# Ryan-Faulkner/Simultaneous-Diffusion-for-Pointclouds

Measured on AMD Instinct MI355X. Metric: Langevin denoising steps/sec on 64×1024 range images, 1/2/4/8 MI355X, higher is better.
Workload: dtype fp32x3; 1 GPU; Line.yml simultaneous sampling step (score-net fwd + Langevin update + consistency merge), 64x1024x2 range images; views_per_gpu=4, megabatch_views=4, mode=viewsplit, conv_arithmetic=fp32x3, parallelism=views1

## Files before the change

### simultaneous-diffusion-for-pointclouds_amd/csrc/conv_kernel.h

```cpp
#pragma once
#include <type_traits>

#include "common.h"

namespace sdp {

#ifndef SDP_KO
#define SDP_KO 0
#endif

#ifndef SDP_DMA_AUX
#define SDP_DMA_AUX 0
#endif
#ifndef SDP_STORE_AUX
#define SDP_STORE_AUX 0
#endif
#ifndef SDP_STORE_AUX16
#define SDP_STORE_AUX16 SDP_STORE_AUX
#endif

#ifndef SDP_S2_RING
#define SDP_S2_RING 4
#endif

#ifdef SDP_TIMING
#define SDP_T(i) do { if (tid == 0) tclk[i] = __builtin_amdgcn_s_memtime(); } while (0)
#else
#define SDP_T(i) do { } while (0)
#endif

constexpr int PSTRIDE = 144;

template <int WM, int TC, int KS, int NW = 4, int NJ = 4, bool IO16 = false>
struct ConvTile {
  static constexpr int NTH = 64 * NW;
  static constexpr int WN = NW / WM;
  static constexpr int RW = 128 / TC;
  static constexpr int TR = WM * RW;
  static constexpr int NTILE = WN * 16 * NJ;
  static constexpr int WPC = 4 * (NJ == 2 ? 2 : 1) / NW;
  static constexpr int HALO = KS == 3 ? 1 : 0;
  static constexpr int PC = TC + 2 * HALO;
  static constexpr int PR = TR + 2 * HALO;
  static constexpr int NPIX = PR * PC;
  static constexpr int UPP = IO16 ? 4 : 8;
  static constexpr int NU = (NPIX * UPP + NTH - 1) / NTH;
  static constexpr int PATCH_BYTES = NU * (NTH / UPP) * PSTRIDE;
  static constexpr int RAW_BYTES = NU * NTH * 16;
  static constexpr int PIPE_BYTES = 2 * PATCH_BYTES + RAW_BYTES;
  static constexpr int EPI_BYTES = WM * 64 * (NTILE + 8) * 4;
  static constexpr int LDS_BYTES = PIPE_BYTES > EPI_BYTES ? PIPE_BYTES : EPI_BYTES;
  static_assert(LDS_BYTES * WPC <= 160 * 1024, "LDS budget (WPC workgroups per CU)");
};

SDP_DEV float4 ld4(const float* p) { return *reinterpret_cast<const float4*>(p); }

template <int NU, int NT, int NSTG_ = 5>
struct XformPlan {
  static constexpr int tap_of(int k) { return k * NT / NU; }
  static constexpr int first(int tap) {
    int k = 0;
    while (k < NU && tap_of(k) < tap) ++k;
    return k;
  }
  static constexpr int count(int tap) {
    int n = 0;
    for (int k = 0; k < NU; ++k) n += tap_of(k) == tap ? 1 : 0;
    return n;
  }
  static constexpr int max_count() {
    int m = 0;
    for (int t = 0; t < NT; ++t) m = count(t) > m ? count(t) : m;
    return m;
  }
  static constexpr int NSTG = NSTG_;
  static constexpr int stage_blk(int q, int Q, int NBLK) { return 2 + q * (NBLK - 2) / (Q > 0 ? Q : 1); }
};

constexpr int s2_pos(int phase, int t) {
  const int rho = phase >> 1, gamma = phase & 1;
  return ((rho ? 0 : 1) + (t >> 1)) * 3 + (gamma ? 0 : 1) + (t & 1);
}

template <int MODE, int WM, int TC, int KS, bool POOL, bool ZP, bool PELU, int SH = 32, int NW = 4, bool TRN = false,
          int NJ = 4, bool IO16 = false, bool S2 = false>
__global__ __launch_bounds__(64 * NW, NJ == 2 ? 2 : 1) void conv_mfma_kernel(ConvArgs a) {
#if defined(__HIP_DEVICE_COMPILE__)
  static_assert(!IO16 || MODE == MODE_BF16, "the bf16 tape runs in bf16 mode");
  constexpr int ES = IO16 ? 2 : 4;
  constexpr int CPU = IO16 ? 8 : 4;
  constexpr int USH = IO16 ? 2 : 3;
  constexpr int PPU = CPU / 2;
  constexpr bool COPY = IO16 && !PELU;
  static_assert((SH == 32) == (MODE == MODE_F32), "bf16 modes: 16x16 shape; exact fp32: 32x32");
  static_assert(NW == 4 || (SH == 16 && !POOL), "2-wave workgroups: the 16x16 non-pooled forward only");
  static_assert(NJ == 4 || (SH == 16 && !POOL && KS == 3 && WM == 1), "32-Cout waves: the 16x16 3x3 tiles only");
  static_assert(!S2 || (NJ == 2 && NW == 4 && TC == 16 && ZP && !TRN && !IO16), "4x4 stride-2: zero-padded 32-Cout-wave tiles");
  using T = ConvTile<WM, TC, KS, NW, NJ, IO16>;
  constexpr int NTH = T::NTH;
  constexpr int NT = S2 ? 4 : KS * KS;
  constexpr bool TRANS = TRN && SH == 16 && !POOL;
  constexpr int NU = T::NU;
  constexpr int XT = NT >= 4 ? 4 : NT;
  __shared__ __attribute__((aligned(16))) char lds[T::LDS_BYTES];
  char* const raw = lds + 2 * T::PATCH_BYTES;

  const int tid = threadIdx.x, lane = tid & 63, wave = tid >> 6;
#ifdef SDP_TIMING
  unsigned long long tclk[8] = {0, 0, 0, 0, 0, 0, 0, 0};
  unsigned long long tbar = 0;
  const unsigned long long rt0 = __builtin_amdgcn_s_memrealtime();
#endif
  SDP_T(0);
  const int wm = WM == 1 ? 0 : (wave & 1), wn = WM == 1 ? wave : (wave >> 1);
  const int d = S2 ? 2 : a.dil, Hs = a.H / d, Ws = a.W / d;
  const int tiles_c = Ws / TC, tiles_rc = (Hs / T::TR) * tiles_c;
  const int nwg = gridDim.x;
  int t = (nwg & 7) ? (int)blockIdx.x : ((int)blockIdx.x & 7) * (nwg >> 3) + ((int)blockIdx.x >> 3);
  const int cblk = a.cpair ? (t & 1) : (int)blockIdx.y;
  if (a.cpair) t >>= 1;
  const int b = t / a.tiles_per_img;
  const int tile = t - b * a.tiles_per_img;
  t = tile;
  const int ph = t / tiles_rc;
  t -= ph * tiles_rc;
  const int ph_r = ph / d, ph_c = ph - (ph / d) * d;
  int trow, tcol;
  if (a.strip_w) {
    const int R = Hs / T::TR, sw = a.strip_w;
    const int strip = t / (R * sw), w_ = t - strip * (R * sw);
    trow = w_ / sw;
    tcol = strip * sw + (w_ - trow * sw);
  } else {
    trow = t / tiles_c;
    tcol = t % tiles_c;
  }
  const int sr0 = trow * T::TR, sc0 = tcol * TC;
  const int n0 = cblk * T::NTILE;
  const int wrow0 = wm * T::RW;

  const int Cin = a.Cin, Cout = a.Cout;
  const int nck = Cin / 32;
  const int nchunks = S2 ? 4 * nck : nck;
  const int NB = Cout / 32;
  const int f0 = n0 / 16 + wn * NJ;
  const int nbg0 = f0 / 2;

  f32x16 acc[4][2];
  f32x4 acc4[8][NJ];
  if constexpr (SH == 32) {
    static_for<0, 4>([&](auto i) {
      static_for<0, 2>([&](auto j) {
#pragma unroll
        for (int r = 0; r < 16; ++r) acc[i][j][r] = 0.f;
      });
    });
  } else {
    static_for<0, 8>([&](auto i) {
      static_for<0, NJ>([&](auto j) {
#pragma unroll
        for (int r = 0; r < 4; ++r) acc4[i][j][r] = 0.f;
      });
    });
  }

  const bool c16 = SH == 16 && a.wf16 != nullptr;
  const __amdgpu_buffer_rsrc_t wrs =
      __builtin_amdgcn_make_buffer_rsrc((void*)(c16 ? a.wf16 : a.wf), 0, 0x7fffffff, 0x00020000);
  const int wv0 = ((nbg0 + 0) * 64 + lane) * 64, wv1 = ((nbg0 + 1) * 64 + lane) * 64;
  typedef __attribute__((ext_vector_type(4))) unsigned u32x4;
  constexpr int NBUF = S2 ? SDP_S2_RING : (NT % 3 == 0) ? 3 : 2;
  uint4 bq[NBUF][NJ / 2][4];
  int wq16[NJ];
  const int wlo16 = __builtin_amdgcn_readfirstlane(c16 ? 1024 : 16);
  {
    const int g = lane >> 4, h = g & 1, sg = g >> 1;
    static_for<0, NJ>([&](auto njc) {
      constexpr int nj = decltype(njc)::value;
      const int L = 16 * (nj & 1) + (lane & 15) + 32 * h;
      wq16[nj] = c16 ? ((f0 + nj) * 128 + lane) * 16 : ((nbg0 + (nj >> 1)) * 64 + L) * 64 + sg * 32;
    });
  }
  auto load_b = [&](auto buf, int chunk, int tap) __attribute__((always_inline)) {
    constexpr int J = decltype(buf)::value;
    if constexpr (SDP_KO & 4) return;
    const int so = __builtin_amdgcn_readfirstlane(((chunk * NT + tap) * NB) * 4096);
    if constexpr (SH == 32) {
      static_for<0, 4>([&](auto q) {
        const u32x4 v0 = __builtin_amdgcn_raw_buffer_load_b128(wrs, wv0 + q * 16, so, 0);
        const u32x4 v1 = __builtin_amdgcn_raw_buffer_load_b128(wrs, wv1 + q * 16, so, 0);
        bq[J][0][q] = make_uint4(v0.x, v0.y, v0.z, v0.w);
        bq[J][1][q] = make_uint4(v1.x, v1.y, v1.z, v1.w);
      });
    } else {
      static_for<0, NJ>([&](auto njc) {
        constexpr int nj = decltype(njc)::value;
        const u32x4 vh = __builtin_amdgcn_raw_buffer_load_b128(wrs, wq16[nj], so, 0);
        bq[J][nj >> 1][2 * (nj & 1)] = make_uint4(vh.x, vh.y, vh.z, vh.w);
        if constexpr (MODE != MODE_BF16) {
          const u32x4 vl = __builtin_amdgcn_raw_buffer_load_b128(wrs, wq16[nj] + wlo16, so, 0);
          bq[J][nj >> 1][2 * (nj & 1) + 1] = make_uint4(vl.x, vl.y, vl.z, vl.w);
        }
      });
    }
  };

  const char* inb = reinterpret_cast<const char*>(a.in) + (size_t)b * a.H * a.W * Cin * ES;
  const float* ssb = a.pro_ss + (size_t)b * a.ss_bstride;
  auto chunk_cc = [&](int c) __attribute__((always_inline)) {
    if constexpr (S2) return (c >= 2 * nck ? c - 2 * nck : c) >> 1;
    else return c;
  };
  auto chunk_soff = [&](int c) __attribute__((always_inline)) {
    if constexpr (S2) {
      c = min(c, nchunks - 1);
      const int rho = c >= 2 * nck ? 1 : 0, r = c - rho * 2 * nck;
      return ((rho * a.W + (r & 1)) * Cin + (r >> 1) * 32) * ES;
    } else {
      return c * 32 * ES;
    }
  };
  const int my_cv = tid & (T::UPP - 1);
  float4 ssv[2][PPU];
  auto load_ss = [&](auto buf, int chunk) __attribute__((always_inline)) {
    constexpr int SB = decltype(buf)::value;
    static_for<0, PPU>([&](auto kc) { ssv[SB][kc] = ld4(ssb + (chunk * 32 + my_cv * CPU) * 2 + 4 * decltype(kc)::value); });
  };

  const __amdgpu_buffer_rsrc_t irs =
      __builtin_amdgcn_make_buffer_rsrc((void*)inb, 0, a.H * a.W * Cin * ES, 0x00020000);
  int uoff[NU];
  unsigned uvalid = 0;
  static_for<0, NU>([&](auto kc) {
    constexpr int k = decltype(kc)::value;
    int u = tid + k * NTH;
    bool valid = u < T::NPIX * T::UPP;
    u = valid ? u : 0;
    const int pix = u >> USH, cv = u & (T::UPP - 1);
    const int pr = pix / T::PC, pc = pix - pr * T::PC;
    int sr = sr0 - T::HALO + pr, sc = sc0 - T::HALO + pc;
    if (a.circular) {
      sr = sr < 0 ? sr + Hs : (sr >= Hs ? sr - Hs : sr);
      sc = sc < 0 ? sc + Ws : (sc >= Ws ? sc - Ws : sc);
    } else {
      valid = valid && sr >= 0 && sr < Hs && sc >= 0 && sc < Ws;
      sr = min(max(sr, 0), Hs - 1);
      sc = min(max(sc, 0), Ws - 1);
    }
    const int y = sr * d + ph_r, x = sc * d + ph_c;
    uoff[k] = ((y * a.W + x) * Cin + cv * CPU) * ES;
    uvalid |= (valid ? 1u : 0u) << k;
  });
  auto load_unit = [&](auto kc, int chunk) __attribute__((always_inline)) {
    constexpr int k = decltype(kc)::value;
    if constexpr (SDP_KO & 1) return;
    const int base = __builtin_amdgcn_readfirstlane(((tid & ~63) + k * NTH) * 16);
    __builtin_amdgcn_raw_ptr_buffer_load_lds(
        irs, reinterpret_cast<__attribute__((address_space(3))) void*>(reinterpret_cast<uintptr_t>(raw + base)), 16,
        uoff[k], chunk_soff(chunk), 0, SDP_DMA_AUX);
  };
  const i32x4 irs_o = buffer_desc(inb, (uint32_t)(a.H * a.W * Cin * ES));
  auto load_unit_o = [&](auto kc, int chunk) __attribute__((always_inline)) {
    constexpr int k = decltype(kc)::value;
    if constexpr (SDP_KO & 1) return;
    const uint32_t base = (uint32_t)(uintptr_t)(raw + ((tid & ~63) + k * NTH) * 16);
    dma16_lds_opaque(irs_o, base, uoff[k], chunk_soff(chunk));
  };
  auto xform_load = [&](auto kc) __attribute__((always_inline)) {
    constexpr int k = decltype(kc)::value;
    return *reinterpret_cast<const float4*>(raw + (tid + k * NTH) * 16);
  };
  auto xform_store = [&](auto kc, auto pb, float4 v) __attribute__((always_inline)) {
    constexpr int k = decltype(kc)::value;
    constexpr int PB = decltype(pb)::value;
    const int pix = (tid + k * NTH) >> USH;
    if constexpr (COPY) {
      uint4 u = __builtin_bit_cast(uint4, v);
      if constexpr (ZP) {
        if (!((uvalid >> k) & 1u)) u = make_uint4(0u, 0u, 0u, 0u);
      }
      *reinterpret_cast<uint4*>(lds + PB * T::PATCH_BYTES + pix * PSTRIDE + my_cv * 16) = u;
      return;
    }
    if constexpr (IO16) {
      const uint4 u = __builtin_bit_cast(uint4, v);
      const float4 lo = bf4_to_f4(make_uint2(u.x, u.y)), hi = bf4_to_f4(make_uint2(u.z, u.w));
      float x8[8] = {lo.x, lo.y, lo.z, lo.w, hi.x, hi.y, hi.z, hi.w};
#pragma unroll
      for (int e = 0; e < 8; ++e) {
        const float4 sv = ssv[PB][e >> 1];
        x8[e] = fmaf(x8[e], (e & 1) ? sv.z : sv.x, (e & 1) ? sv.w : sv.y);
        if constexpr (PELU) x8[e] = elu_max(x8[e]);
        if constexpr (ZP) {
          if (!((uvalid >> k) & 1u)) x8[e] = 0.f;
        }
      }
      *reinterpret_cast<uint4*>(lds + PB * T::PATCH_BYTES + pix * PSTRIDE + my_cv * 16) =
          make_uint4(pack_bf2(x8[0], x8[1]), pack_bf2(x8[2], x8[3]), pack_bf2(x8[4], x8[5]), pack_bf2(x8[6], x8[7]));
      return;
    }
    const float4 ssv0 = ssv[PB][0], ssv1 = ssv[PB][1];
    v.x = fmaf(v.x, ssv0.x, ssv0.y);
    v.y = fmaf(v.y, ssv0.z, ssv0.w);
    v.z = fmaf(v.z, ssv1.x, ssv1.y);
    v.w = fmaf(v.w, ssv1.z, ssv1.w);
    if constexpr (PELU) {
      v.x = elu_max(v.x); v.y = elu_max(v.y); v.z = elu_max(v.z); v.w = elu_max(v.w);
    }
    if constexpr (ZP) {
      if (!((uvalid >> k) & 1u)) v = make_float4(0.f, 0.f, 0.f, 0.f);
    }
    char* dst = lds + PB * T::PATCH_BYTES + pix * PSTRIDE;
    if constexpr (MODE == MODE_F32) {
      *reinterpret_cast<float4*>(dst + my_cv * 16) = v;
    } else {
      bf16x4 hi;
      hi[0] = (__bf16)v.x; hi[1] = (__bf16)v.y; hi[2] = (__bf16)v.z; hi[3] = (__bf16)v.w;
      *reinterpret_cast<bf16x4*>(dst + my_cv * 8) = hi;
      if constexpr (MODE == MODE_F32X3) {
        bf16x4 lo;
        lo[0] = (__bf16)(v.x - (float)hi[0]);
        lo[1] = (__bf16)(v.y - (float)hi[1]);
        lo[2] = (__bf16)(v.z - (float)hi[2]);
        lo[3] = (__bf16)(v.w - (float)hi[3]);
        *reinterpret_cast<bf16x4*>(dst + 64 + my_cv * 8) = lo;
      }
    }
  };
  auto xform_unit = [&](auto kc, auto pb) __attribute__((always_inline)) { xform_store(kc, pb, xform_load(kc)); };
  auto xform_piece = [&](auto kc, auto hc, auto pb, float4 v4) __attribute__((always_inline)) {
    constexpr int k = decltype(kc)::value, h = decltype(hc)::value, PB = decltype(pb)::value;
    if constexpr (SDP_KO & 2) return;
    const int pix = (tid + k * NTH) >> USH;
    float x0, x1;
    if constexpr (IO16) {
      const uint32_t w = __float_as_uint(h == 0 ? v4.x : h == 1 ? v4.y : h == 2 ? v4.z : v4.w);
      x0 = __uint_as_float(w << 16);
      x1 = __uint_as_float(w & 0xffff0000u);
    } else {
      x0 = h ? v4.z : v4.x;
      x1 = h ? v4.w : v4.y;
    }
    const float4 sv = ssv[PB][h];
    x0 = fmaf(x0, sv.x, sv.y);
    x1 = fmaf(x1, sv.z, sv.w);
    if constexpr (PELU) {
      x0 = elu_max(x0);
      x1 = elu_max(x1);
    }
    if constexpr (ZP) {
      const bool ok = (uvalid >> k) & 1u;
      x0 = ok ? x0 : 0.f;
      x1 = ok ? x1 : 0.f;
    }
    typedef __attribute__((ext_vector_type(2))) __bf16 bf16x2;
    bf16x2 hi;
    hi[0] = (__bf16)x0;
    hi[1] = (__bf16)x1;
    char* dst = lds + PB * T::PATCH_BYTES + pix * PSTRIDE + my_cv * (2 * CPU) + h * 4;
    *reinterpret_cast<bf16x2*>(dst) = hi;
    if constexpr (MODE == MODE_F32X3) {
      bf16x2 lo;
      lo[0] = (__bf16)(x0 - (float)hi[0]);
      lo[1] = (__bf16)(x1 - (float)hi[1]);
      *reinterpret_cast<bf16x2*>(dst + 64) = lo;
    }
  };

  SDP_T(1);
  load_b(std::integral_constant<int, 0>{}, 0, 0);
  static_for<1, NBUF - 1>([&](auto j) { load_b(j, 0, decltype(j)::value); });
  load_ss(std::integral_constant<int, 0>{}, 0);
  static_for<0, NU>([&](auto k) { load_unit(k, 0); });
  static_for<0, NU>([&](auto k) { xform_unit(k, std::integral_constant<int, 0>{}); });
  if (nchunks > 1) {
    load_ss(std::integral_constant<int, 1>{}, chunk_cc(1));
    static_for<0, NU>([&](auto k) { load_unit(k, 1); });
  }
  __syncthreads();
  SDP_T(2);

  const int a_lane_off16 = (lane & 15) * PSTRIDE + (lane >> 4) * 16;
  auto read_a = [&](const char* pat, auto tap_c, auto s_c, bf16x8* hi, bf16x8* lo) __attribute__((always_inline)) {
    constexpr int tap = decltype(tap_c)::value, s = decltype(s_c)::value;
    constexpr int kh = (KS == 3) ? tap / 3 : 0, kw = (KS == 3) ? tap % 3 : 0;
    static_for<0, 4>([&](auto mbc) {
      constexpr int i = decltype(mbc)::value, mb = 4 * s + i;
      constexpr int mr = mb / (TC / 16), mc = (mb % (TC / 16)) * 16;
      const char* src = pat + ((wrow0 + mr + kh) * T::PC + mc + kw) * PSTRIDE + a_lane_off16;
      hi[i] = *reinterpret_cast<const bf16x8*>(src);
      if constexpr (MODE == MODE_F32X3) lo[i] = *reinterpret_cast<const bf16x8*>(src + 64);
    });
  };

  auto do_chunk = [&](auto parity, int chunk) __attribute__((always_inline)) {
    constexpr int P = decltype(parity)::value;
    const char* pat = lds + P * T::PATCH_BYTES;
    bf16x8 pre_hi[4], pre_lo[4];
    if constexpr (MODE != MODE_F32) read_a(pat, std::integral_constant<int, 0>{}, std::integral_constant<int, 0>{},
                                           pre_hi, pre_lo);
    static_for<0, NT>([&](auto tap_c) {
      constexpr int tap = decltype(tap_c)::value;
      constexpr int DIST = NBUF - 1;
      constexpr int CUR = NBUF >= 3 ? tap % NBUF : (tap + P) & 1;
      constexpr int NXT = NBUF >= 3 ? (tap + DIST) % NBUF : (tap + 1 + P) & 1;
      if constexpr (tap + DIST < NT) load_b(std::integral_constant<int, NXT>{}, chunk, tap + DIST);
      else load_b(std::integral_constant<int, NXT>{}, min(chunk + 1, nchunks - 1), tap + DIST - NT);
      __builtin_amdgcn_sched_barrier(0);
      constexpr int NX = (tap < XT) ? (NU - tap + XT - 1) / XT : 0;
      float4 xv[NX > 0 ? NX : 1];
      auto xform_loads = [&]() __attribute__((always_inline)) {
        static_for<0, NX>([&](auto j) { xv[j] = xform_load(std::integral_constant<int, tap + XT * j>{}); });
      };
      auto xform_stores = [&]() __attribute__((always_inline)) {
        static_for<0, NX>([&](auto j) {
          xform_store(std::integral_constant<int, tap + XT * j>{}, std::integral_constant<int, 1 - P>{}, xv[j]);
        });
      };
      auto dmas = [&]() __attribute__((always_inline)) {
        if constexpr (tap == NT - 1) load_ss(std::integral_constant<int, P>{}, min(chunk + 2, nchunks - 1));
        static_for<0, NU>([&](auto kc) {
          constexpr int dt = NT > XT ? XT : 0;
          if constexpr (dt == tap) load_unit(kc, chunk + 2);
        });
      };
      if constexpr (MODE == MODE_F32) {
        xform_loads();
        xform_stores();
        if constexpr (NT == 1) __builtin_amdgcn_sched_barrier(0);
        dmas();
        const int kh = (KS == 3) ? tap / 3 : 0, kw = (KS == 3) ? tap % 3 : 0;
#pragma unroll
        for (int half = 0; half < 2; ++half) {
          float av[4][8];
          static_for<0, 4>([&](auto mbc) {
            constexpr int mb = decltype(mbc)::value;
            constexpr int mr = mb / (TC / 32), mc = (mb % (TC / 32)) * 32;
            const int pix = (wrow0 + mr + kh) * T::PC + mc + (lane & 31) + kw;
            const char* src = pat + pix * PSTRIDE + (lane >> 5) * 64 + half * 32;
            const float4 f0 = *reinterpret_cast<const float4*>(src);
            const float4 f1 = *reinterpret_cast<const float4*>(src + 16);
            av[mb][0] = f0.x; av[mb][1] = f0.y; av[mb][2] = f0.z; av[mb][3] = f0.w;
            av[mb][4] = f1.x; av[mb][5] = f1.y; av[mb][6] = f1.z; av[mb][7] = f1.w;
          });
#pragma unroll
          for (int kk = 0; kk < 8; ++kk) {
            const int k = half * 8 + kk;
            static_for<0, 2>([&](auto nbc) {
              constexpr int nb = decltype(nbc)::value;
              const uint4 bv = bq[CUR][nb][k >> 2];
              const uint32_t bw = (k & 3) == 0 ? bv.x : (k & 3) == 1 ? bv.y : (k & 3) == 2 ? bv.z : bv.w;
              const float bf = __uint_as_float(bw);
              static_for<0, 4>([&](auto mbc) {
                constexpr int mb = decltype(mbc)::value;
                acc[mb][nb] = __builtin_amdgcn_mfma_f32_32x32x2f32(av[mb][kk], bf, acc[mb][nb], 0, 0, 0);
              });
            });
          }
        }
      } else {
        float4 xv[NX > 0 ? NX : 1];
        static_for<0, NX>([&](auto j) { xv[j] = xform_load(std::integral_constant<int, tap + XT * j>{}); });
        bf16x8 c0_hi[4], c0_lo[4], c1_hi[4], c1_lo[4];
        static_for<0, 4>([&](auto mb) {
          c0_hi[mb] = pre_hi[mb];
          if constexpr (MODE == MODE_F32X3) c0_lo[mb] = pre_lo[mb];
        });
        read_a(pat, tap_c, std::integral_constant<int, 1>{}, c1_hi, c1_lo);
        if constexpr (tap + 1 < NT)
          read_a(pat, std::integral_constant<int, tap + 1>{}, std::integral_constant<int, 0>{}, pre_hi, pre_lo);
        if constexpr (NT > 1) dmas();
        constexpr int NBLK = 8 * NJ;
        static_for<0, NBLK>([&](auto blk_c) {
          constexpr int blk = decltype(blk_c)::value;
          {
            constexpr int s = blk / (4 * NJ), nj = (blk / 4) % NJ, i = blk & 3, mb = 4 * s + i;
            const uint4 h4 = bq[CUR][nj >> 1][2 * (nj & 1)], l4 = bq[CUR][nj >> 1][2 * (nj & 1) + 1];
            const bf16x8 bhi = *reinterpret_cast<const bf16x8*>(&h4);
            const bf16x8 blo = *reinterpret_cast<const bf16x8*>(&l4);
            const bf16x8 ahi = s == 0 ? c0_hi[i] : c1_hi[i];
            if constexpr (TRANS) {
              if constexpr (MODE == MODE_F32X3) {
                const bf16x8 alo = s == 0 ? c0_lo[i] : c1_lo[i];
                acc4[mb][nj] = __builtin_amdgcn_mfma_f32_16x16x32_bf16(bhi, alo, acc4[mb][nj], 0, 0, 0);
                acc4[mb][nj] = __builtin_amdgcn_mfma_f32_16x16x32_bf16(blo, ahi, acc4[mb][nj], 0, 0, 0);
              }
              acc4[mb][nj] = __builtin_amdgcn_mfma_f32_16x16x32_bf16(bhi, ahi, acc4[mb][nj], 0, 0, 0);
            } else {
              if constexpr (MODE == MODE_F32X3) {
                const bf16x8 alo = s == 0 ? c0_lo[i] : c1_lo[i];
                acc4[mb][nj] = __builtin_amdgcn_mfma_f32_16x16x32_bf16(alo, bhi, acc4[mb][nj], 0, 0, 0);
                acc4[mb][nj] = __builtin_amdgcn_mfma_f32_16x16x32_bf16(ahi, blo, acc4[mb][nj], 0, 0, 0);
              }
              acc4[mb][nj] = __builtin_amdgcn_mfma_f32_16x16x32_bf16(ahi, bhi, acc4[mb][nj], 0, 0, 0);
            }
          }
          if constexpr (COPY) {
            if constexpr (blk < NX) xform_store(std::integral_constant<int, tap + XT * blk>{}, std::integral_constant<int, 1 - P>{},
                                                xv[blk]);
          } else if constexpr (blk < PPU * NX) {
            xform_piece(std::integral_constant<int, tap + XT * (blk / PPU)>{}, std::integral_constant<int, blk % PPU>{},
                        std::integral_constant<int, 1 - P>{}, xv[blk / PPU]);
          }
          __builtin_amdgcn_sched_barrier(0);
        });
        if constexpr (NT == 1) dmas();
      }
    });
#ifdef SDP_TIMING
    const unsigned long long tb0 = __builtin_amdgcn_s_memtime();
#endif
    __builtin_amdgcn_s_waitcnt(0xc07f);
    if constexpr (!(SDP_KO & 8)) __builtin_amdgcn_s_barrier();
#ifdef SDP_TIMING
    tbar += __builtin_amdgcn_s_memtime() - tb0;
#endif
  };
  using XP = XformPlan<NU, NT, (MODE == MODE_BF16 && !IO16 && !S2) ? 8 : 5>;
  constexpr int NQ = MODE == MODE_F32X3 ? 8 : 4;
  constexpr int NWL = NJ * (MODE == MODE_F32X3 ? 2 : 1);
  constexpr int NBLK = 8 * NJ;
  static_assert(NQ <= NBLK / 2 && 2 * NWL <= NBLK, "the tap's fillers fit its blocks");
  using I0 = std::integral_constant<int, 0>;
  using I1 = std::integral_constant<int, 1>;
  auto read_a1 = [&](const char* pat, auto pos_c, auto s_c, auto i_c, auto lo_c) __attribute__((always_inline)) {
    constexpr int pos = decltype(pos_c)::value, s = decltype(s_c)::value, i = decltype(i_c)::value;
    constexpr int kh = pos / 3, kw = pos % 3, mb = 4 * s + i;
    constexpr int mr = mb / (TC / 16), mc = (mb % (TC / 16)) * 16;
    return *reinterpret_cast<const bf16x8*>(pat + ((wrow0 + mr + kh) * T::PC + mc + kw) * PSTRIDE + a_lane_off16 +
                                            (decltype(lo_c)::value ? 64 : 0));
  };
  auto load_b1 = [&](auto buf, auto q_c, int chunk, int tap) __attribute__((always_inline)) {
    constexpr int J = decltype(buf)::value, q = decltype(q_c)::value;
    constexpr int nj = MODE == MODE_F32X3 ? (q >> 1) : q, part = MODE == MODE_F32X3 ? (q & 1) : 0;
    if constexpr (SDP_KO & 4) return;
    const int so = __builtin_amdgcn_readfirstlane(((chunk * NT + tap) * NB) * 4096 + (part ? wlo16 : 0));
    const u32x4 v = __builtin_amdgcn_raw_buffer_load_b128(wrs, wq16[nj], so, 0);
    bq[J][nj >> 1][2 * (nj & 1) + part] = make_uint4(v.x, v.y, v.z, v.w);
  };
  auto do_chunk9 = [&](auto parity, auto phase_c, int chunk) __attribute__((always_inline)) {
    constexpr int P = decltype(parity)::value, PHS = decltype(phase_c)::value;
    const char* pat = lds + P * T::PATCH_BYTES;
    bf16x8 ca[2][4], cb[2][4];
    static_for<0, 4>([&](auto i) {
      using POS0 = std::integral_constant<int, S2 ? s2_pos(PHS, 0) : 0>;
      ca[0][i] = read_a1(pat, POS0{}, I0{}, i, I0{});
      if constexpr (MODE == MODE_F32X3) ca[1][i] = read_a1(pat, POS0{}, I0{}, i, I1{});
    });
    load_ss(std::integral_constant<int, P>{}, chunk_cc(min(chunk + 2, nchunks - 1)));
    static_for<0, NT>([&](auto tap_c) {
      constexpr int tap = decltype(tap_c)::value;
      constexpr int DIST = NBUF - 1;
      constexpr int CUR = tap % NBUF, NXT = (tap + DIST) % NBUF;
      using POS = std::integral_constant<int, S2 ? s2_pos(PHS, tap) : tap>;
      using POSN = std::integral_constant<int, S2 ? s2_pos(PHS, tap + 1 < NT ? tap + 1 : 0) : tap + 1>;
      constexpr int U0 = XP::first(tap), UN = XP::count(tap), Q = COPY ? UN : UN * PPU * XP::NSTG;
      constexpr int UNA = UN > 0 ? UN : 1;
      const int wchunk = tap + DIST < NT ? chunk : min(chunk + 1, nchunks - 1);
      constexpr int wtap = tap + DIST < NT ? tap + DIST : tap + DIST - NT;
      float4 xr[UNA];
      float py0[PPU * UNA], py1[PPU * UNA], pe0[PPU * UNA], pe1[PPU * UNA];
      uint32_t phi[PPU * UNA], plo[PPU * UNA];
      auto stage = [&](auto pc_c, auto st_c) __attribute__((always_inline)) {
        constexpr int pc = decltype(pc_c)::value, st = decltype(st_c)::value;
        constexpr int j = pc / PPU, h = pc % PPU, k = U0 + j, PB = 1 - P;
        if constexpr (SDP_KO & 2) return;
        if constexpr (COPY) {
          xform_store(std::integral_constant<int, U0 + decltype(pc_c)::value>{}, std::integral_constant<int, PB>{},
                      xr[decltype(pc_c)::value]);
          return;
        }
        auto raw2 = [&](float& r0, float& r1) __attribute__((always_inline)) {
          const float4 v = xr[j];
          if constexpr (IO16) {
            const uint32_t w = __float_as_uint(h == 0 ? v.x : h == 1 ? v.y : h == 2 ? v.z : v.w);
            r0 = __uint_as_float(w << 16);
            r1 = __uint_as_float(w & 0xffff0000u);
          } else {
            r0 = h ? v.z : v.x;
            r1 = h ? v.w : v.y;
          }
        };
        if constexpr (XP::NSTG == 8) {
          const float4 v = xr[j];
          const float4 sv = ssv[PB][h];
          if constexpr (st == 0) {
            py0[pc] = fmaf(h ? v.z : v.x, sv.x, sv.y);
            if constexpr (PELU) pe0[pc] = fminf(py0[pc], 0.f);
          } else if constexpr (st == 1) {
            py1[pc] = fmaf(h ? v.w : v.y, sv.z, sv.w);
            if constexpr (PELU) pe1[pc] = fminf(py1[pc], 0.f);
          } else if constexpr (st == 2) {
            if constexpr (PELU) pe0[pc] = __expf(pe0[pc]);
          } else if constexpr (st == 3) {
            if constexpr (PELU) pe1[pc] = __expf(pe1[pc]);
          } else if constexpr (st == 4) {
            if constexpr (PELU) py0[pc] = fmaxf(py0[pc], pe0[pc] - 1.0f);
            if constexpr (ZP) py0[pc] = ((uvalid >> k) & 1u) ? py0[pc] : 0.f;
          } else if constexpr (st == 5) {
            if constexpr (PELU) py1[pc] = fmaxf(py1[pc], pe1[pc] - 1.0f);
            if constexpr (ZP) py1[pc] = ((uvalid >> k) & 1u) ? py1[pc] : 0.f;
          } else if constexpr (st == 6) {
            typedef __attribute__((ext_vector_type(2))) __bf16 bf16x2;
            bf16x2 hi;
            hi[0] = (__bf16)py0[pc];
            hi[1] = (__bf16)py1[pc];
            phi[pc] = *reinterpret_cast<const uint32_t*>(&hi);
          } else {
            const int pix = (tid + k * NTH) >> 3;
            *reinterpret_cast<uint32_t*>(lds + PB * T::PATCH_BYTES + pix * PSTRIDE + my_cv * 8 + h * 4) = phi[pc];
          }
          return;
        }
        if constexpr (st == 0) {
          float r0, r1;
          raw2(r0, r1);
          const float4 sv = ssv[PB][h];
          py0[pc] = fmaf(r0, sv.x, sv.y);
          py1[pc] = fmaf(r1, sv.z, sv.w);
          if constexpr (PELU) {
            pe0[pc] = fminf(py0[pc], 0.f);
            pe1[pc] = fminf(py1[pc], 0.f);
          }
        } else if constexpr (st == 1) {
          if constexpr (PELU) {
            pe0[pc] = __expf(pe0[pc]);
            pe1[pc] = __expf(pe1[pc]);
          }
        } else if constexpr (st == 2) {
          if constexpr (PELU) {
            py0[pc] = fmaxf(py0[pc], pe0[pc] - 1.0f);
            py1[pc] = fmaxf(py1[pc], pe1[pc] - 1.0f);
          }
          if constexpr (ZP) {
            const bool ok = (uvalid >> k) & 1u;
            py0[pc] = ok ? py0[pc] : 0.f;
            py1[pc] = ok ? py1[pc] : 0.f;
          }
        } else if constexpr (st == 3) {
          typedef __attribute__((ext_vector_type(2))) __bf16 bf16x2;
          bf16x2 hi;
          hi[0] = (__bf16)py0[pc];
          hi[1] = (__bf16)py1[pc];
          phi[pc] = *reinterpret_cast<const uint32_t*>(&hi);
          if constexpr (MODE == MODE_F32X3) {
            bf16x2 lo;
            lo[0] = (__bf16)(py0[pc] - (float)hi[0]);
            lo[1] = (__bf16)(py1[pc] - (float)hi[1]);
            plo[pc] = *reinterpret_cast<const uint32_t*>(&lo);
          }
        } else {
          const int pix = (tid + k * NTH) >> USH;
          char* dst = lds + PB * T::PATCH_BYTES + pix * PSTRIDE + my_cv * (2 * CPU) + h * 4;
          *reinterpret_cast<uint32_t*>(dst) = phi[pc];
          if constexpr (MODE == MODE_F32X3) *reinterpret_cast<uint32_t*>(dst + 64) = plo[pc];
        }
      };
      static_for<0, NBLK>([&](auto blk_c) {
        constexpr int blk = decltype(blk_c)::value;
        constexpr int s = blk / (4 * NJ), nj = (blk / 4) % NJ, i = blk & 3, mb = 4 * s + i;
        if constexpr (blk < UN) xr[blk] = xform_load(std::integral_constant<int, U0 + blk>{});
        {
          const uint4 h4 = bq[CUR][nj >> 1][2 * (nj & 1)], l4 = bq[CUR][nj >> 1][2 * (nj & 1) + 1];
          const bf16x8 bhi = *reinterpret_cast<const bf16x8*>(&h4);
          const bf16x8 blo = *reinterpret_cast<const bf16x8*>(&l4);
          const bf16x8 ahi = s == 0 ? ca[0][i] : cb[0][i];
          if constexpr (TRANS) {
            if constexpr (MODE == MODE_F32X3) {
              const bf16x8 alo = s == 0 ? ca[1][i] : cb[1][i];
              acc4[mb][nj] = __builtin_amdgcn_mfma_f32_16x16x32_bf16(bhi, alo, acc4[mb][nj], 0, 0, 0);
              acc4[mb][nj] = __builtin_amdgcn_mfma_f32_16x16x32_bf16(blo, ahi, acc4[mb][nj], 0, 0, 0);
            }
            acc4[mb][nj] = __builtin_amdgcn_mfma_f32_16x16x32_bf16(bhi, ahi, acc4[mb][nj], 0, 0, 0);
          } else {
            if constexpr (MODE == MODE_F32X3) {
              const bf16x8 alo = s == 0 ? ca[1][i] : cb[1][i];
              acc4[mb][nj] = __builtin_amdgcn_mfma_f32_16x16x32_bf16(alo, bhi, acc4[mb][nj], 0, 0, 0);
              acc4[mb][nj] = __builtin_amdgcn_mfma_f32_16x16x32_bf16(ahi, blo, acc4[mb][nj], 0, 0, 0);
            }
            acc4[mb][nj] = __builtin_amdgcn_mfma_f32_16x16x32_bf16(ahi, bhi, acc4[mb][nj], 0, 0, 0);
          }
        }
        if constexpr (blk < NQ) {
          constexpr int q = blk, ii = MODE == MODE_F32X3 ? (q >> 1) : q, lo = MODE == MODE_F32X3 ? (q & 1) : 0;
          cb[lo][ii] = read_a1(pat, POS{}, I1{}, std::integral_constant<int, ii>{}, std::integral_constant<int, lo>{});
        }
        if constexpr ((blk & 1) && (blk >> 1) < NWL)
          load_b1(std::integral_constant<int, NXT>{}, std::integral_constant<int, (blk >> 1)>{}, wchunk, wtap);
        if constexpr (tap + 1 < NT && blk >= NBLK / 2 && blk < NBLK / 2 + NQ) {
          constexpr int q = blk - NBLK / 2, ii = MODE == MODE_F32X3 ? (q >> 1) : q, lo = MODE == MODE_F32X3 ? (q & 1) : 0;
          ca[lo][ii] = read_a1(pat, POSN{}, I0{}, std::integral_constant<int, ii>{},
                               std::integral_constant<int, lo>{});
        }
        static_for<0, Q>([&](auto q_c) {
          constexpr int q = decltype(q_c)::value;
          if constexpr (XP::stage_blk(q, Q, NBLK) == blk) {
            if constexpr (COPY) stage(std::integral_constant<int, q>{}, std::integral_constant<int, 0>{});
            else stage(std::integral_constant<int, q / XP::NSTG>{}, std::integral_constant<int, q % XP::NSTG>{});
          }
        });
        if constexpr (UN > 0 && blk >= NBLK - UN)
          load_unit_o(std::integral_constant<int, U0 + blk - (NBLK - UN)>{}, chunk + 2);
        __builtin_amdgcn_sched_barrier(0);
      });
    });
    __builtin_amdgcn_s_waitcnt(0xc07f);
    if constexpr (!(SDP_KO & 8)) __builtin_amdgcn_s_barrier();
  };
  static_assert(NT % 2 == 1 || (S2 && NT % NBUF == 0), "weight-ring slots repeat from chunk to chunk");
#ifndef SDP_DGRAD16_TAPS
#define SDP_DGRAD16_TAPS 0
#endif
  if constexpr (S2) {
    static_assert(MODE != MODE_F32 && NT % NBUF == 0, "4x4 stride-2: the tap schedule of the bf16 modes");
    static_assert(XP::max_count() * PPU * XP::NSTG <= 2 * (NBLK - 2), "at most two transform stages per block");
    for (int chunk = 0; chunk < 2 * nck; chunk += 2) {
      do_chunk9(I0{}, I0{}, chunk);
      do_chunk9(I1{}, I1{}, chunk + 1);
    }
    for (int chunk = 2 * nck; chunk < nchunks; chunk += 2) {
      do_chunk9(I0{}, std::integral_constant<int, 2>{}, chunk);
      do_chunk9(I1{}, std::integral_constant<int, 3>{}, chunk + 1);
    }
  } else if constexpr (MODE != MODE_F32 && NT == 9 && (!TRANS || (IO16 && SDP_DGRAD16_TAPS))) {
    static_assert(XP::max_count() * PPU * XP::NSTG <= 2 * (NBLK - 2), "at most two transform stages per block");
    for (int chunk = 0; chunk < nchunks; chunk += 2) {
      do_chunk9(I0{}, I0{}, chunk);
      do_chunk9(I1{}, I0{}, chunk + 1);
    }
  } else {
    for (int chunk = 0; chunk < nchunks; chunk += 2) {
      do_chunk(std::integral_constant<int, 0>{}, chunk);
      do_chunk(std::integral_constant<int, 1>{}, chunk + 1);
    }
  }

  SDP_T(3);
  if (TRANS && (!a.dact || TC < 32 || NW != 4)) {
    if constexpr (TRANS) {
    __builtin_amdgcn_s_waitcnt(0);
    const int Ho = a.H, Wo = a.W;
    const size_t bo = (size_t)b * Ho * Wo * Cout;
    const int img_bytes = Ho * Wo * Cout * ES;
    auto rs = [&](const float* p) {
      return __builtin_amdgcn_make_buffer_rsrc((void*)(reinterpret_cast<const char*>(p) + bo * ES), 0, img_bytes, 0x00020000);
    };
    const int lq = lane >> 4, lcol = lane & 15;
    constexpr int CB = TC / 16;
    const int voff = (lcol * d * Cout + 4 * lq) * ES;
    auto soff = [&](int mb, int nj) {
      const int mr = mb / CB, mc = (mb % CB) * 16;
      const int y = (sr0 + wrow0 + mr) * d + ph_r, x = (sc0 + mc) * d + ph_c;
      return __builtin_amdgcn_readfirstlane(((y * Wo + x) * Cout + n0 + wn * 16 * NJ + nj * 16) * ES);
    };
    auto ld = [&](__amdgpu_buffer_rsrc_t r, int so) {
      if constexpr (IO16) {
        typedef __attribute__((ext_vector_type(2))) unsigned u32x2;
        const u32x2 q = __builtin_amdgcn_raw_buffer_load_b64(r, voff, so, 0);
        return bf4_to_f4(make_uint2(q.x, q.y));
      } else {
        const u32x4 q = __builtin_amdgcn_raw_buffer_load_b128(r, voff, so, 0);
        return make_float4(__uint_as_float(q.x), __uint_as_float(q.y), __uint_as_float(q.z), __uint_as_float(q.w));
      }
    };
    auto st = [&](float4 v, __amdgpu_buffer_rsrc_t r, int so, auto aux_c) {
      constexpr int AUX = decltype(aux_c)::value;
      if constexpr (IO16) {
        typedef __attribute__((ext_vector_type(2))) unsigned u32x2;
        const uint2 w = f4_to_bf4(v);
        __builtin_amdgcn_raw_buffer_store_b64(u32x2{w.x, w.y}, r, voff, so, AUX);
      } else {
        const u32x4 q = {__float_as_uint(v.x), __float_as_uint(v.y), __float_as_uint(v.z), __float_as_uint(v.w)};
        __builtin_amdgcn_raw_buffer_store_b128(q, r, voff, so, AUX);
      }
    };
    auto rs_or_out = [&](const float* p) { return rs(p ? p : a.out); };
    const __amdgpu_buffer_rsrc_t ors = rs(a.out), xrs = rs_or_out(a.aux), rrs = rs_or_out(a.res), o2rs = rs_or_out(a.out2),
                                 r2rs = rs_or_out(a.res2);
    static_for<0, NJ>([&](auto njc) {
      constexpr int nj = decltype(njc)::value;
      __builtin_amdgcn_sched_barrier(0);
      const int co0 = n0 + wn * 16 * NJ + nj * 16 + 4 * lq;
      float4 hq[8], rq[8], s0 = make_float4(1.f, 0.f, 1.f, 0.f), s1 = s0;
      if (a.dact) static_for<0, 8>([&](auto mb) { hq[mb] = ld(xrs, soff(mb, nj)); });
      if (a.dact == 3) {
        s0 = ld4(a.epi_ss + ((size_t)b * Cout + co0) * 2);
        s1 = ld4(a.epi_ss + ((size_t)b * Cout + co0) * 2 + 4);
      }
      if (a.res) static_for<0, 8>([&](auto mb) { rq[mb] = ld(rrs, soff(mb, nj)); });
      const float4 bias4 = a.bias ? ld4(a.bias + co0) : make_float4(0.f, 0.f, 0.f, 0.f);
      const float4 esc = make_float4(s0.x, s0.z, s1.x, s1.z), esh = make_float4(s0.y, s0.w, s1.y, s1.w);
      float4 v[8];
      static_for<0, 8>([&](auto mbc) {
        constexpr int mb = decltype(mbc)::value;
        const f32x4 q = acc4[mb][nj];
        v[mb] = make_float4(q[0] + bias4.x, q[1] + bias4.y, q[2] + bias4.z, q[3] + bias4.w);
      });
      if (a.up) {
        const int Hi = a.H / 2, Wi = a.W / 2;
        const float shh = (float)(Hi - 1) / (float)(a.H - 1), sww = (float)(Wi - 1) / (float)(a.W - 1);
        const size_t ub = (size_t)b * Hi * Wi * Cout + co0;
        auto lup = [&](size_t e) { return IO16 ? ldg4(reinterpret_cast<const __bf16*>(a.up), e) : ldg4(a.up, e); };
#pragma unroll
        for (int mb = 0; mb < 8; ++mb) {
          const int mr = mb / CB, mc = (mb % CB) * 16;
          const int y = (sr0 + wrow0 + mr) * d + ph_r, x = (sc0 + mc + lcol) * d + ph_c;
          const float fy = shh * (float)y, fx = sww * (float)x;
          const int y0 = (int)fy, x0 = (int)fx;
          const int yp = y0 < Hi - 1 ? 1 : 0, xp = x0 < Wi - 1 ? 1 : 0;
          const float ly1 = fy - (float)y0, ly0 = 1.f - ly1, lx1 = fx - (float)x0, lx0 = 1.f - lx1;
          const float4 v00 = lup(ub + ((size_t)y0 * Wi + x0) * Cout), v01 = lup(ub + ((size_t)y0 * Wi + x0 + xp) * Cout);
          const float4 v10 = lup(ub + ((size_t)(y0 + yp) * Wi + x0) * Cout);
          const float4 v11 = lup(ub + ((size_t)(y0 + yp) * Wi + x0 + xp) * Cout);
          auto bil = [&](float a00, float a01, float a10, float a11) {
            return ly0 * (lx0 * a00 + lx1 * a01) + ly1 * (lx0 * a10 + lx1 * a11);
          };
          v[mb].x = v[mb].x + bil(v00.x, v01.x, v10.x, v11.x);
          v[mb].y = v[mb].y + bil(v00.y, v01.y, v10.y, v11.y);
          v[mb].z = v[mb].z + bil(v00.z, v01.z, v10.z, v11.z);
          v[mb].w = v[mb].w + bil(v00.w, v01.w, v10.w, v11.w);
        }
      }
      if (a.dact) {
        static_for<0, 8>([&](auto mbc) {
          constexpr int mb = decltype(mbc)::value;
          float4 h = hq[mb];
          if (a.dact == 3) h = make_float4(fmaf(h.x, esc.x, esh.x), fmaf(h.y, esc.y, esh.y), fmaf(h.z, esc.z, esh.z),
                                           fmaf(h.w, esc.w, esh.w));
          v[mb] = make_float4(v[mb].x * elu_grad(h.x, a.dact), v[mb].y * elu_grad(h.y, a.dact),
                              v[mb].z * elu_grad(h.z, a.dact), v[mb].w * elu_grad(h.w, a.dact));
        });
      }
      if (a.res) {
        static_for<0, 8>([&](auto mbc) {
          constexpr int mb = decltype(mbc)::value;
          const float4 r = rq[mb];
          v[mb] = make_float4(r.x + v[mb].x, r.y + v[mb].y, r.z + v[mb].z, r.w + v[mb].w);
        });
      }
      if (a.out2) {
        static_for<0, 8>([&](auto mbc) {
          constexpr int mb = decltype(mbc)::value;
// ... 557 lines not shown
```

Before: 383.5 image-steps/s.

## Reuse 3x3 conv A-fragments across vertical taps via register row ring

Adds a row-ring of A-fragment registers for 3x3 16x16 NJ=2 conv tiles. Taps are reordered column-major (kw outer, kh inner) so each LDS patch row is read once per kw column and reused across the three vertical taps. A constexpr check verifies the ring schedule. This targets redundant LDS reads of A operands, at the cost of more live VGPRs (an 18-fragment ring), which risks spills or lower occupancy. Separately, the scale/shift prologue loads and FMAs are now skipped when PELU is off.

```diff
diff --git a/simultaneous-diffusion-for-pointclouds_amd/csrc/conv_kernel.h b/simultaneous-diffusion-for-pointclouds_amd/csrc/conv_kernel.h
--- a/simultaneous-diffusion-for-pointclouds_amd/csrc/conv_kernel.h
+++ b/simultaneous-diffusion-for-pointclouds_amd/csrc/conv_kernel.h
@@ -21,6 +21,10 @@
 
 #ifndef SDP_S2_RING
 #define SDP_S2_RING 4
+#endif
+
+#ifndef SDP_ROWS
+#define SDP_ROWS 1
 #endif
 
 #ifdef SDP_TIMING
@@ -82,6 +86,48 @@
   return ((rho ? 0 : 1) + (t >> 1)) * 3 + (gamma ? 0 : 1) + (t & 1);
 }
 
+constexpr int ROWS_SLOTS = 9;
+constexpr int rows_pos(int o) { return (o % 3) * 3 + o / 3; }
+constexpr int rows_slot(int kw, int row) { return (row + kw) % ROWS_SLOTS; }
+constexpr int rows_read(int o, int blk) {
+  const int kh = o % 3, kw = o / 3, lo = blk & 1;
+  if (kh == 0) {
+    if (kw == 0 && blk < 10) return 4 * (4 + blk / 2) + 2 * lo;
+    if (kw > 0 && blk < 4) return 4 * (7 + blk / 2) + 2 * lo;
+    if (blk == 10 || blk == 11) return 4 * 9 + 2 * lo;
+  } else if (kh == 1) {
+    if (kw < 2 && (blk == 8 || blk == 10)) return 4 * 0 + 2 * (blk == 10 ? 1 : 0) + 1;
+  } else {
+    if (kw < 2 && blk >= 4) return 4 * (1 + (blk - 4) / 2) + 2 * lo + 1;
+  }
+  return -1;
+}
+constexpr bool rows_plan_ok() {
+  for (int kw = 0; kw < 3; ++kw)
+    for (int row = 0; row < 10; ++row)
+      for (int lo = 0; lo < 2; ++lo) {
+        int n = (kw == 0 && row < 4) ? 1 : 0, at = -1;
+        for (int o = 0; o < 9; ++o)
+          for (int blk = 0; blk < 16; ++blk) {
+            const int c = rows_read(o, blk);
+            if (c >= 0 && o / 3 + (c & 1) == kw && c / 4 == row && ((c >> 1) & 1) == lo) {
+              ++n;
+              at = 16 * o + blk;
+            }
+          }
+        if (n != 1) return false;
+        const int kh0 = row > 7 ? row - 7 : 0, mb0 = row - kh0;
+        if (at >= 16 * (3 * kw + kh0) + (mb0 < 4 ? mb0 : 4 + mb0)) return false;
+        const int pkw = row == 9 ? kw : kw - 1, prow = row == 9 ? 0 : row + 1;
+        if (pkw < 0) continue;
+        if (rows_slot(pkw, prow) != rows_slot(kw, row)) return false;
+        const int kh1 = prow < 2 ? prow : 2, mb1 = prow - kh1;
+        if (at < 16 * (3 * pkw + kh1) + (mb1 < 4 ? 4 + mb1 : 8 + mb1)) return false;
+      }
+  return true;
+}
+static_assert(rows_plan_ok(), "A-fragment ring: a row is read once, between its slot's last use and its own first");
+
 template <int MODE, int WM, int TC, int KS, bool POOL, bool ZP, bool PELU, int SH = 32, int NW = 4, bool TRN = false,
           int NJ = 4, bool IO16 = false, bool S2 = false>
 __global__ __launch_bounds__(64 * NW, NJ == 2 ? 2 : 1) void conv_mfma_kernel(ConvArgs a) {
@@ -102,6 +148,7 @@
   constexpr bool TRANS = TRN && SH == 16 && !POOL;
   constexpr int NU = T::NU;
   constexpr int XT = NT >= 4 ? 4 : NT;
+  constexpr bool ROWS = SDP_ROWS && SH == 16 && !S2 && NT == 9 && TC == 16 && NJ == 2 && !TRANS;
   __shared__ __attribute__((aligned(16))) char lds[T::LDS_BYTES];
   char* const raw = lds + 2 * T::PATCH_BYTES;
 
@@ -224,6 +271,7 @@
   float4 ssv[2][PPU];
   auto load_ss = [&](auto buf, int chunk) __attribute__((always_inline)) {
     constexpr int SB = decltype(buf)::value;
+    if constexpr (!PELU) return;
     static_for<0, PPU>([&](auto kc) { ssv[SB][kc] = ld4(ssb + (chunk * 32 + my_cv * CPU) * 2 + 4 * decltype(kc)::value); });
   };
 
@@ -288,9 +336,10 @@
       float x8[8] = {lo.x, lo.y, lo.z, lo.w, hi.x, hi.y, hi.z, hi.w};
 #pragma unroll
       for (int e = 0; e < 8; ++e) {
-        const float4 sv = ssv[PB][e >> 1];
-        x8[e] = fmaf(x8[e], (e & 1) ? sv.z : sv.x, (e & 1) ? sv.w : sv.y);
-        if constexpr (PELU) x8[e] = elu_max(x8[e]);
+        if constexpr (PELU) {
+          const float4 sv = ssv[PB][e >> 1];
+          x8[e] = elu_max(fmaf(x8[e], (e & 1) ? sv.z : sv.x, (e & 1) ? sv.w : sv.y));
+        }
         if constexpr (ZP) {
           if (!((uvalid >> k) & 1u)) x8[e] = 0.f;
         }
@@ -299,12 +348,12 @@
           make_uint4(pack_bf2(x8[0], x8[1]), pack_bf2(x8[2], x8[3]), pack_bf2(x8[4], x8[5]), pack_bf2(x8[6], x8[7]));
       return;
     }
-    const float4 ssv0 = ssv[PB][0], ssv1 = ssv[PB][1];
-    v.x = fmaf(v.x, ssv0.x, ssv0.y);
-    v.y = fmaf(v.y, ssv0.z, ssv0.w);
-    v.z = fmaf(v.z, ssv1.x, ssv1.y);
-    v.w = fmaf(v.w, ssv1.z, ssv1.w);
     if constexpr (PELU) {
+      const float4 ssv0 = ssv[PB][0], ssv1 = ssv[PB][1];
+      v.x = fmaf(v.x, ssv0.x, ssv0.y);
+      v.y = fmaf(v.y, ssv0.z, ssv0.w);
+      v.z = fmaf(v.z, ssv1.x, ssv1.y);
+      v.w = fmaf(v.w, ssv1.z, ssv1.w);
       v.x = elu_max(v.x); v.y = elu_max(v.y); v.z = elu_max(v.z); v.w = elu_max(v.w);
     }
     if constexpr (ZP) {
@@ -341,12 +390,10 @@
       x0 = h ? v4.z : v4.x;
       x1 = h ? v4.w : v4.y;
     }
-    const float4 sv = ssv[PB][h];
-    x0 = fmaf(x0, sv.x, sv.y);
-    x1 = fmaf(x1, sv.z, sv.w);
     if constexpr (PELU) {
-      x0 = elu_max(x0);
-      x1 = elu_max(x1);
+      const float4 sv = ssv[PB][h];
+      x0 = elu_max(fmaf(x0, sv.x, sv.y));
+      x1 = elu_max(fmaf(x1, sv.z, sv.w));
     }
     if constexpr (ZP) {
       const bool ok = (uvalid >> k) & 1u;
@@ -369,7 +416,7 @@
 
   SDP_T(1);
   load_b(std::integral_constant<int, 0>{}, 0, 0);
-  static_for<1, NBUF - 1>([&](auto j) { load_b(j, 0, decltype(j)::value); });
+  static_for<1, NBUF - 1>([&](auto j) { load_b(j, 0, ROWS ? rows_pos(decltype(j)::value) : decltype(j)::value); });
   load_ss(std::integral_constant<int, 0>{}, 0);
   static_for<0, NU>([&](auto k) { load_unit(k, 0); });
   static_for<0, NU>([&](auto k) { xform_unit(k, std::integral_constant<int, 0>{}); });
@@ -542,10 +589,20 @@
     constexpr int P = decltype(parity)::value, PHS = decltype(phase_c)::value;
     const char* pat = lds + P * T::PATCH_BYTES;
     bf16x8 ca[2][4], cb[2][4];
+    bf16x8 ar[2][ROWS ? ROWS_SLOTS : 1];
+    auto read_row = [&](auto kw_c, auto row_c, auto lo_c) __attribute__((always_inline)) {
+      return *reinterpret_cast<const bf16x8*>(pat + ((wrow0 + decltype(row_c)::value) * T::PC + decltype(kw_c)::value) * PSTRIDE +
+                                              a_lane_off16 + (decltype(lo_c)::value ? 64 : 0));
+    };
     static_for<0, 4>([&](auto i) {
-      using POS0 = std::integral_constant<int, S2 ? s2_pos(PHS, 0) : 0>;
-      ca[0][i] = read_a1(pat, POS0{}, I0{}, i, I0{});
-      if constexpr (MODE == MODE_F32X3) ca[1][i] = read_a1(pat, POS0{}, I0{}, i, I1{});
+      if constexpr (ROWS) {
+        ar[0][rows_slot(0, i)] = read_row(I0{}, i, I0{});
+        if constexpr (MODE == MODE_F32X3) ar[1][rows_slot(0, i)] = read_row(I0{}, i, I1{});
+      } else {
+        using POS0 = std::integral_constant<int, S2 ? s2_pos(PHS, 0) : 0>;
+        ca[0][i] = read_a1(pat, POS0{}, I0{}, i, I0{});
+        if constexpr (MODE == MODE_F32X3) ca[1][i] = read_a1(pat, POS0{}, I0{}, i, I1{});
+      }
     });
     load_ss(std::integral_constant<int, P>{}, chunk_cc(min(chunk + 2, nchunks - 1)));
     static_for<0, NT>([&](auto tap_c) {
@@ -557,7 +614,8 @@
       constexpr int U0 = XP::first(tap), UN = XP::count(tap), Q = COPY ? UN : UN * PPU * XP::NSTG;
       constexpr int UNA = UN > 0 ? UN : 1;
       const int wchunk = tap + DIST < NT ? chunk : min(chunk + 1, nchunks - 1);
-      constexpr int wtap = tap + DIST < NT ? tap + DIST : tap + DIST - NT;
+      constexpr int wnext = tap + DIST < NT ? tap + DIST : tap + DIST - NT;
+      constexpr int wtap = ROWS ? rows_pos(wnext) : wnext;
       float4 xr[UNA];
       float py0[PPU * UNA], py1[PPU * UNA], pe0[PPU * UNA], pe1[PPU * UNA];
       uint32_t phi[PPU * UNA], plo[PPU * UNA];
@@ -583,13 +641,18 @@
         };
         if constexpr (XP::NSTG == 8) {
           const float4 v = xr[j];
-          const float4 sv = ssv[PB][h];
           if constexpr (st == 0) {
-            py0[pc] = fmaf(h ? v.z : v.x, sv.x, sv.y);
-            if constexpr (PELU) pe0[pc] = fminf(py0[pc], 0.f);
+            py0[pc] = h ? v.z : v.x;
+            if constexpr (PELU) {
+              py0[pc] = fmaf(py0[pc], ssv[PB][h].x, ssv[PB][h].y);
+              pe0[pc] = fminf(py0[pc], 0.f);
+            }
           } else if constexpr (st == 1) {
-            py1[pc] = fmaf(h ? v.w : v.y, sv.z, sv.w);
-            if constexpr (PELU) pe1[pc] = fminf(py1[pc], 0.f);
+            py1[pc] = h ? v.w : v.y;
+            if constexpr (PELU) {
+              py1[pc] = fmaf(py1[pc], ssv[PB][h].z, ssv[PB][h].w);
+              pe1[pc] = fminf(py1[pc], 0.f);
+            }
           } else if constexpr (st == 2) {
             if constexpr (PELU) pe0[pc] = __expf(pe0[pc]);
           } else if constexpr (st == 3) {
@@ -615,10 +678,12 @@
         if constexpr (st == 0) {
           float r0, r1;
           raw2(r0, r1);
-          const float4 sv = ssv[PB][h];
-          py0[pc] = fmaf(r0, sv.x, sv.y);
-          py1[pc] = fmaf(r1, sv.z, sv.w);
+          py0[pc] = r0;
+          py1[pc] = r1;
           if constexpr (PELU) {
+            const float4 sv = ssv[PB][h];
+            py0[pc] = fmaf(r0, sv.x, sv.y);
+            py1[pc] = fmaf(r1, sv.z, sv.w);
             pe0[pc] = fminf(py0[pc], 0.f);
             pe1[pc] = fminf(py1[pc], 0.f);
           }
@@ -664,30 +729,40 @@
           const uint4 h4 = bq[CUR][nj >> 1][2 * (nj & 1)], l4 = bq[CUR][nj >> 1][2 * (nj & 1) + 1];
           const bf16x8 bhi = *reinterpret_cast<const bf16x8*>(&h4);
           const bf16x8 blo = *reinterpret_cast<const bf16x8*>(&l4);
-          const bf16x8 ahi = s == 0 ? ca[0][i] : cb[0][i];
+          auto afrag = [&](auto lo_c) __attribute__((always_inline)) {
+            constexpr int lo = decltype(lo_c)::value;
+            if constexpr (ROWS) return ar[lo][rows_slot(tap / 3, mb + tap % 3)];
+            else return s == 0 ? ca[lo][i] : cb[lo][i];
+          };
+          const bf16x8 ahi = afrag(I0{});
           if constexpr (TRANS) {
             if constexpr (MODE == MODE_F32X3) {
-              const bf16x8 alo = s == 0 ? ca[1][i] : cb[1][i];
+              const bf16x8 alo = afrag(I1{});
               acc4[mb][nj] = __builtin_amdgcn_mfma_f32_16x16x32_bf16(bhi, alo, acc4[mb][nj], 0, 0, 0);
               acc4[mb][nj] = __builtin_amdgcn_mfma_f32_16x16x32_bf16(blo, ahi, acc4[mb][nj], 0, 0, 0);
             }
             acc4[mb][nj] = __builtin_amdgcn_mfma_f32_16x16x32_bf16(bhi, ahi, acc4[mb][nj], 0, 0, 0);
           } else {
             if constexpr (MODE == MODE_F32X3) {
-              const bf16x8 alo = s == 0 ? ca[1][i] : cb[1][i];
+              const bf16x8 alo = afrag(I1{});
               acc4[mb][nj] = __builtin_amdgcn_mfma_f32_16x16x32_bf16(alo, bhi, acc4[mb][nj], 0, 0, 0);
               acc4[mb][nj] = __builtin_amdgcn_mfma_f32_16x16x32_bf16(ahi, blo, acc4[mb][nj], 0, 0, 0);
             }
             acc4[mb][nj] = __builtin_amdgcn_mfma_f32_16x16x32_bf16(ahi, bhi, acc4[mb][nj], 0, 0, 0);
           }
         }
-        if constexpr (blk < NQ) {
+        if constexpr (ROWS) {
+          constexpr int c = rows_read(tap, blk);
+          if constexpr (c >= 0 && (MODE == MODE_F32X3 || !(c & 2)))
+            ar[(c >> 1) & 1][rows_slot(tap / 3 + (c & 1), c / 4)] = read_row(std::integral_constant<int, tap / 3 + (c & 1)>{}, std::integral_constant<int, c / 4>{},
+                                               std::integral_constant<int, (c >> 1) & 1>{});
+        } else if constexpr (blk < NQ) {
           constexpr int q = blk, ii = MODE == MODE_F32X3 ? (q >> 1) : q, lo = MODE == MODE_F32X3 ? (q & 1) : 0;
           cb[lo][ii] = read_a1(pat, POS{}, I1{}, std::integral_constant<int, ii>{}, std::integral_constant<int, lo>{});
         }
         if constexpr ((blk & 1) && (blk >> 1) < NWL)
           load_b1(std::integral_constant<int, NXT>{}, std::integral_constant<int, (blk >> 1)>{}, wchunk, wtap);
-        if constexpr (tap + 1 < NT && blk >= NBLK / 2 && blk < NBLK / 2 + NQ) {
+        if constexpr (!ROWS && tap + 1 < NT && blk >= NBLK / 2 && blk < NBLK / 2 + NQ) {
           constexpr int q = blk - NBLK / 2, ii = MODE == MODE_F32X3 ? (q >> 1) : q, lo = MODE == MODE_F32X3 ? (q & 1) : 0;
           ca[lo][ii] = read_a1(pat, POSN{}, I0{}, std::integral_constant<int, ii>{},
                                std::integral_constant<int, lo>{});
```

After: 396.3 image-steps/s (median of 6 runs). 3.4% higher.
